# Livioni/OmniVGGT-official

Measured on AMD Instinct MI355X. Metric: frames/sec (518^2, S views) aggregator hot path, higher is better.
Workload: dtype bf16

## Files before the change

### omnivggt-official_amd/build.py

```python
import hashlib
import os
import subprocess
import sys
from concurrent.futures import ThreadPoolExecutor

HERE = os.path.dirname(os.path.abspath(__file__))
CSRC = os.path.join(HERE, "csrc")
OUT = os.path.join(HERE, "libomnivggt_hip.so")
SOURCES = ["ovg_gemm.hip", "ovg_attn.hip", "ovg_elem.hip", "ovg_block.hip", "ovg_head.hip", "ovg_camhead.hip", "ovg_camtab.hip"]
FLAGS = ["--offload-arch=gfx950", "-O3", "-std=c++17", "-fPIC", "-fno-gpu-rdc", "-Wall", "-Wno-unused-function"]
EXTRA_FLAGS = {"ovg_attn.hip": ["-fno-honor-nans"]}


PINNED_ATTENTION_KERNELS = {"IDF16bLi4ELi8ELi0ELi2ELb0ELi5ELi0E": 4, "IDF16bLi4ELi4ELi0ELi2ELb0ELi3ELi0E": 4, "IDF16bLi2ELi4ELi0ELi2ELb0ELi3ELi0E": 2}


PINNED_LOOP_MNEMONICS = {"v_mfma_f32_16x16x32_bf16", "v_exp_f32", "v_cvt_pk_bf16_f32", "ds_read_b128",
                         "v_add_u32_e32", "v_or_b32_e32", "v_lshl_or_b32", "v_lshl_add_u32", "v_add_lshl_u32", "v_lshlrev_b32_e32", "v_and_b32_e32"}


def check_pinned_attention_loops(asm_text):
    import re
    kernels, name, body = {}, None, []
    for line in asm_text.splitlines():
        m = re.match(r"^(_ZN\S*attn16_kernel\S*):", line)
        if m:
            name, body = m.group(1), []
            continue
        if name is not None:
            body.append(line)
            if "s_endpgm" in line:
                kernels[name], name = body, None
    report = {}
    for pat, qb in PINNED_ATTENTION_KERNELS.items():
        hits = [k for k in kernels if pat in k]
        if len(hits) != 1:
            raise RuntimeError("pinned-attention check: kernel %s not found exactly once (%r)" % (pat, hits))
        blocks, cur = [], []
        for line in kernels[hits[0]]:
            if re.match(r"^\.LBB", line):
                blocks.append(cur)
                cur = []
            elif line.startswith("\t") and not line.strip().startswith((".", ";")):
                cur.append(line.split()[0])
        blocks.append(cur)
        pinned = [b for b in blocks if sum("v_mfma" in i for i in b) == 18 * qb and b.count("v_exp_f32") == 16 * qb]
        if len(pinned) != 1:
            raise RuntimeError("pinned-attention check: %s has %d candidate hot loops (MFMA / exp counts per block: %r)"
                               % (pat, len(pinned), [(sum("v_mfma" in i for i in b), b.count("v_exp_f32")) for b in blocks if any("v_mfma" in i for i in b)]))
        hot = pinned[0]
        if hot.count("v_cvt_pk_bf16_f32") != 8 * qb or hot.count("ds_read_b128") != 16:
            raise RuntimeError("pinned-attention check: %s hot loop holds %d converts / %d fragment reads" % (pat, hot.count("v_cvt_pk_bf16_f32"), hot.count("ds_read_b128")))
        bad = [i for i in hot if not (i.startswith("s_") or i in PINNED_LOOP_MNEMONICS)]
        if bad:
            raise RuntimeError("pinned-attention check: hipcc put instructions outside the pinned tile's own set (register copies / spills / "
                               "re-materialised operands) inside the hot loop of %s: %r -- the bf16 attention results of such a build are NOT "
                               "trustworthy" % (pat, sorted(set(bad))))
        report[pat] = {"instructions": len(hot), "mfma": 18 * qb}
    return report

TRANS_OPS = ("v_exp_f32", "v_log_f32", "v_rcp_f32", "v_rsq_f32", "v_sqrt_f32", "v_sin_f32", "v_cos_f32", "v_exp_f16", "v_log_f16", "v_rcp_f16", "v_rsq_f16", "v_sqrt_f16")


def _vregs(operand):
    import re
    out = set()
    for m in re.finditer(r"\bv\[(\d+):(\d+)\]", operand):
        out.update(range(int(m.group(1)), int(m.group(2)) + 1))
    for m in re.finditer(r"\bv(\d+)\b", operand):
        out.add(int(m.group(1)))
    return out


def check_trans_use_in_asm(asm_text):
    seen, in_asm, prev = 0, False, None
    for line in asm_text.splitlines():
        t = line.strip()
        if t.startswith(";;#ASMSTART"):
            in_asm = True
            continue
        if t.startswith(";;#ASMEND"):
            in_asm = False
            continue
        if not line.startswith("\t") or not t or t.startswith((".", ";")):
            if t.endswith(":"):
                prev = None
            continue
        mnem, _, rest = t.partition(" ")
        ops = [o.strip() for o in rest.split(",")]
        if in_asm and prev is not None and (mnem.startswith("v_") or mnem.startswith("ds_") or mnem.startswith("global_") or mnem.startswith("buffer_")):
            seen += 1
            srcs = set()
            for o in (ops[1:] if mnem.startswith("v_") and not mnem.startswith("v_cmp") else ops):
                srcs |= _vregs(o)
            if mnem.startswith("v_fma_mix") or mnem.startswith("v_pk_add") or mnem.startswith("v_mfma"):
                srcs |= _vregs(ops[0])
            if srcs & prev[1]:
                raise RuntimeError("trans-use check: compiler-scheduled %s writes v%s and the inline-asm `%s` directly behind it reads it -- "
                                   "hipcc pads no hazard for asm statements; put an opaque wait state between them (ovg_attn16.h pv_step)"
                                   % (prev[0], sorted(prev[1]), t))
        if mnem == "s_nop":
            prev = None
            continue
        if not in_asm and mnem.split("_e32")[0].split("_e64")[0] in TRANS_OPS:
            prev = (mnem, _vregs(ops[0]))
        else:
            prev = None
    return seen


def _hipcc():
    for c in (os.environ.get("HIPCC"), "/opt/rocm/bin/hipcc", "hipcc"):
        if c and (os.path.isabs(c) and os.path.exists(c) or not os.path.isabs(c)):
            return c
    raise RuntimeError("hipcc not found")


def _digest():
    h = hashlib.sha256()
    files = [os.path.join(CSRC, f) for f in sorted(os.listdir(CSRC))]
    files.append(os.path.join(HERE, "..", "include", "omnivggt_hip.h"))
    for f in files:
        with open(f, "rb") as fh:
            h.update(fh.read())
    h.update(" ".join(FLAGS).encode())
    h.update(repr(sorted(EXTRA_FLAGS.items())).encode())
    return h.hexdigest()


def is_current():
    stamp = OUT + ".stamp"
    return os.path.exists(OUT) and os.path.exists(stamp) and open(stamp).read().strip() == _digest()


def have_hipcc():
    try:
        c = _hipcc()
    except RuntimeError:
        return False
    import shutil
    return os.path.isabs(c) or shutil.which(c) is not None


def build(force=False, verbose=True):
    import fcntl
    import shutil
    import tempfile
    stamp = OUT + ".stamp"
    with open(OUT + ".lock", "w") as lock:
        fcntl.flock(lock, fcntl.LOCK_EX)
        try:
            dig = _digest()
            if not force and is_current():
                return OUT
            hipcc = _hipcc()
            os.makedirs(os.path.join(HERE, "build"), exist_ok=True)
            objdir = tempfile.mkdtemp(prefix="obj.", dir=os.path.join(HERE, "build"))

            def cc(src, extra=()):
                obj = os.path.join(objdir, src.replace(".hip", ".o"))
                cmd = [hipcc, *FLAGS, *EXTRA_FLAGS.get(src, []), *extra, "-c", os.path.join(CSRC, src), "-o", obj]
                if src == "ovg_attn.hip":
                    cmd.insert(1, "-save-temps=obj")
                r = subprocess.run(cmd, capture_output=True, text=True)
                if r.returncode != 0:
                    raise RuntimeError("hipcc failed for %s:\n%s" % (src, r.stderr[-4000:]))
                if verbose and r.stderr.strip():
                    sys.stderr.write(r.stderr)
                if src == "ovg_attn.hip" and not extra:
                    asm = [f for f in os.listdir(objdir) if f.startswith("ovg_attn") and f.endswith(".s") and "gfx950" in f]
                    if len(asm) != 1:
                        raise RuntimeError("pinned-attention check: expected one gfx950 assembly file of ovg_attn.hip, found %r" % asm)
                    try:
                        text = open(os.path.join(objdir, asm[0])).read()
                        check_pinned_attention_loops(text)
                        check_trans_use_in_asm(text)
                    except RuntimeError as e:
                        sys.stderr.write("WARNING: %s\nWARNING: rebuilding ovg_attn.hip with -DOVG_ATTN_PIPE_LOOP=0 (compiler-scheduled attention "
                                         "tile body: correct, slower); fix csrc/ovg_attn16_body_q*.inc for this compiler to get the pinned loop back\n" % e)
                        return cc(src, extra=("-DOVG_ATTN_PIPE_LOOP=0",))
                return obj

            try:
                with ThreadPoolExecutor(max_workers=len(SOURCES)) as ex:
                    objs = list(ex.map(cc, SOURCES))
                tmp_out = os.path.join(objdir, "libomnivggt_hip.so")
                r = subprocess.run([hipcc, "--offload-arch=gfx950", "-shared", "-fPIC", "-o", tmp_out, *objs], capture_output=True, text=True)
                if r.returncode != 0:
                    raise RuntimeError("link failed:\n" + r.stderr[-4000:])
                if os.path.exists(stamp):
                    os.remove(stamp)
                os.replace(tmp_out, OUT)
                with open(stamp + ".tmp", "w") as fh:
                    fh.write(dig)
                os.replace(stamp + ".tmp", stamp)
            finally:
                shutil.rmtree(objdir, ignore_errors=True)
            return OUT
        finally:
            fcntl.flock(lock, fcntl.LOCK_UN)


if __name__ == "__main__":
    print(build(force="--force" in sys.argv))
```

### omnivggt-official_amd/csrc/ovg_gemm.hip

```cpp
#include "ovg_common.h"
#include <mutex>
#include <type_traits>
#include <utility>
#include <vector>

namespace {

constexpr int BM = 128, BN = 128;

#ifdef OVG_GEMM_TIMELINE
__device__ unsigned long long* g_tl_buf = nullptr;
__device__ int g_tl_stagger = 0;
OVG_DEV void tl_mark(int slot) {
  if ((threadIdx.x & 63) != 0 || g_tl_buf == nullptr) return;
  const int wave = threadIdx.x >> 6, last = (blockDim.x >> 6) - 1;
  if (wave != 0 && wave != last) return;
  unsigned long long* row = g_tl_buf + (size_t)blockIdx.x * 16 + (wave == 0 ? 0 : 8);
  row[slot] = wall_clock64();
  if (slot == 0) { row[4] = __builtin_amdgcn_s_getreg((31 << 11) | 4); row[5] = __builtin_amdgcn_s_getreg((31 << 11) | 20); row[6] = clock64(); }
  if (slot == 3) row[7] = clock64();
}
OVG_DEV void tl_stagger() {
  if (g_tl_stagger <= 0 || blockIdx.x >= 256) return;
  const unsigned long long until = wall_clock64() + (unsigned long long)(((blockIdx.x >> 3) & 7) * g_tl_stagger);
// ... 350 lines not shown
        if (m < M) *reinterpret_cast<u32x4*>(static_cast<T*>(p.y) + (int64_t)m * p.ldy + n_w0 + pch * 8) = t[j];
      }
    }
  }
}

template <typename T, int EPI, bool OUT_F32, int MT, int XP = 0, bool X3 = false>
OVG_DEV void linear_epilogue(const ovg_linear_params& p, const f32x4 (&acc)[4][MT], const int m_w0, const int n_w0, const int row_lim = -1) {
  if constexpr (EPI == OVG_EPI_RES) {
    if (p.inject != nullptr) { linear_epilogue_impl<T, EPI, OUT_F32, MT, true, XP, X3>(p, acc, m_w0, n_w0, row_lim); return; }
  }
  linear_epilogue_impl<T, EPI, OUT_F32, MT, false, XP, X3>(p, acc, m_w0, n_w0, row_lim);
}

template <typename T, int EPI, bool OUT_F32, int MT, int XP, bool X3 = false>
OVG_DEV void linear_epilogue_auto(const ovg_linear_params& p, const f32x4 (&acc)[4][MT], const int m_w0, const int n_w0, unsigned char* img) {
  if constexpr (!XP && sizeof(T) == 2) {
    if constexpr ((EPI == OVG_EPI_STORE || EPI == OVG_EPI_GELU) && !OUT_F32 && !X3) {
      if (((p.ldy * (int64_t)sizeof(T)) & 15) == 0) { linear_epilogue_staged<T, EPI, MT>(p, acc, m_w0, n_w0, img); return; }
    }
    if constexpr (EPI == OVG_EPI_RES) {
      bool inj_here = false;
      if (p.inject != nullptr) {
        const int rem = m_w0 % (int)p.inj_period;
        inj_here = rem == 0 || (int)p.inj_period - rem < 16 * MT;
      }
      if (!inj_here) { linear_epilogue_staged<T, EPI, MT>(p, acc, m_w0, n_w0, img); return; }
    }
  }
  linear_epilogue<T, EPI, OUT_F32, MT, XP, X3>(p, acc, m_w0, n_w0);
}


template <typename T, int EPI, bool OUT_F32, int XP = 0, bool X3 = false>
__global__ __launch_bounds__(256, 2) void linear_kernel(ovg_linear_params p, int ntiles_n) {
  __shared__ __attribute__((aligned(16))) unsigned char lds[2 * 128 * 128];
  const int M = (int)p.M, N = (int)p.N, K = (int)p.K;
  int tm, tn;
  tl_stagger();
  tl_mark(0);
  tile_coords(xcd_remap(blockIdx.x, gridDim.x), (M + BM - 1) / BM, ntiles_n, tm, tn);
  const int m0 = tm * BM, n0 = tn * BN;
  f32x4 acc[4][4];
  gemm_mainloop<T, false, X3>(static_cast<const T*>(p.x), p.ldx, static_cast<const T*>(p.w), p.ldw, M, N, K, m0, n0, lds, acc,
                              static_cast<const T*>(p.x_lo), static_cast<const T*>(p.w_lo));
  tl_mark(2);
  const int wave = __builtin_amdgcn_readfirstlane(threadIdx.x >> 6);
  linear_epilogue_auto<T, EPI, OUT_F32, 4, XP, X3>(p, acc, m0 + (wave & 1) * 64, n0 + (wave >> 1) * 64, lds + wave * 8192);
  tl_mark(3);
}

template <typename T, int MT, bool NORM, bool ROPE, bool X3 = false>
OVG_DEV void qk_rows(const f32x4 (&acc)[4][MT], const float* __restrict__ nw_p, const float* __restrict__ nb_p,
                     const float* __restrict__ rope_cos, const float* __restrict__ rope_sin, T* __restrict__ out, const int64_t npad,
                     const int m_w0, const int M, const int seq, const int h, const int tokens_per_view, const int n_special,
                     const int grid_w, const float qk_eps, const float scale, unsigned char* img = nullptr, T* __restrict__ out_lo = nullptr) {
  const int lane = threadIdx.x & 63, g = lane >> 4, lr = lane & 15;
  const FastDiv div_seq(seq), div_tpv(ROPE ? tokens_per_view : 1), div_gw(ROPE ? grid_w : 1);
  float nw[16], nb[16];
  if constexpr (NORM) {
#pragma unroll
    for (int nt = 0; nt < 4; ++nt) {
      const f32x4 a = *reinterpret_cast<const f32x4*>(nw_p + nt * 16 + 4 * g);
      const f32x4 b = *reinterpret_cast<const f32x4*>(nb_p + nt * 16 + 4 * g);
#pragma unroll
      for (int r = 0; r < 4; ++r) { nw[nt * 4 + r] = a[r]; nb[nt * 4 + r] = b[r]; }
    }
  }
#pragma unroll
  for (int mt = 0; mt < MT; ++mt) {
    const int m = m_w0 + mt * 16 + lr;
    const bool valid = m < M;
    const int mm = valid ? m : M - 1;
    int bidx, n;
    div_seq.divmod(mm, bidx, n);
    f32x4 cy, sy, cx, sxn;
    if constexpr (ROPE) {
      int vw, t, py, px;
      div_tpv.divmod(mm, vw, t);
      const int pp = t - n_special;
      div_gw.divmod(pp >= 0 ? pp : 0, py, px);
      py = pp >= 0 ? py + 1 : 0;
      px = pp >= 0 ? px + 1 : 0;
      cy = *reinterpret_cast<const f32x4*>(rope_cos + py * 16 + 4 * g);
      sy = *reinterpret_cast<const f32x4*>(rope_sin + py * 16 + 4 * g);
      cx = *reinterpret_cast<const f32x4*>(rope_cos + px * 16 + 4 * g);
      sxn = *reinterpret_cast<const f32x4*>(rope_sin + px * 16 + 4 * g);
    }
    float v[16];
#pragma unroll
    for (int nt = 0; nt < 4; ++nt)
#pragma unroll
      for (int r = 0; r < 4; ++r) v[nt * 4 + r] = acc[nt][mt][r];
    if constexpr (NORM) {
      float s = 0.f;
#pragma unroll
      for (int i = 0; i < 16; ++i) s += v[i];
      s = quad16_sum(s);
      const float mean = s * (1.0f / 64.0f);
      float q = 0.f;
#pragma unroll
      for (int i = 0; i < 16; ++i) { const float d = v[i] - mean; q += d * d; }
      q = quad16_sum(q);
      float rstd;
      if constexpr (sizeof(T) == 4 || X3) rstd = 1.0f / sqrtf(q * (1.0f / 64.0f) + qk_eps);
      else rstd = __builtin_amdgcn_rsqf(q * (1.0f / 64.0f) + qk_eps);
#pragma unroll
      for (int i = 0; i < 16; ++i) v[i] = (v[i] - mean) * rstd * nw[i] + nb[i];
    }
    if constexpr (ROPE) {
#pragma unroll
      for (int r = 0; r < 4; ++r) {
        const float a0 = v[r], a1 = v[4 + r];
        v[r] = a0 * cy[r] - a1 * sy[r];
        v[4 + r] = a1 * cy[r] + a0 * sy[r];
        const float b0 = v[8 + r], b1 = v[12 + r];
        v[8 + r] = b0 * cx[r] - b1 * sxn[r];
        v[12 + r] = b1 * cx[r] + b0 * sxn[r];
      }
    }
#pragma unroll
    for (int i = 0; i < 16; ++i) v[i] *= scale;
    if constexpr (sizeof(T) == 2) {
      if (img != nullptr) {
#pragma unroll
        for (int nt = 0; nt < 4; ++nt) stage16_put4<T>(img, mt * 16 + lr, nt * 16 + 4 * g, v[nt * 4], v[nt * 4 + 1], v[nt * 4 + 2], v[nt * 4 + 3]);
        continue;
      }
    }
    if (valid) {
      const int64_t off = (((int64_t)bidx * OVG_H + h) * npad + n) * OVG_D + 4 * g;
      T* dst = out + off;
#pragma unroll
      for (int nt = 0; nt < 4; ++nt) {
        if constexpr (X3) store4_hilo(dst + nt * 16, out_lo + off + nt * 16, v[nt * 4], v[nt * 4 + 1], v[nt * 4 + 2], v[nt * 4 + 3]);
        else store4<T>(dst + nt * 16, v[nt * 4], v[nt * 4 + 1], v[nt * 4 + 2], v[nt * 4 + 3]);
      }
    }
  }
  if constexpr (sizeof(T) == 2) {
    if (img != nullptr) {
      const int prow = lane >> 3, pch = lane & 7;
#pragma unroll
      for (int i0 = 0; i0 < 2 * MT; i0 += 4) {
        u32x4 t[4];
#pragma unroll
        for (int j = 0; j < 4; ++j) t[j] = stage16_get(img, (i0 + j) * 8 + prow, pch);
#pragma unroll
        for (int j = 0; j < 4; ++j) {
          const int m = m_w0 + (i0 + j) * 8 + prow;
          int bidx, n;
          div_seq.divmod(m < M ? m : M - 1, bidx, n);
          if (m < M) *reinterpret_cast<u32x4*>(out + (((int64_t)bidx * OVG_H + h) * npad + n) * OVG_D + pch * 8) = t[j];
        }
      }
    }
  }
}

template <typename T, int MT, bool X3 = false>
OVG_DEV void qk_epilogue(const ovg_qkv_params& p, f32x4 (&acc)[4][MT], const int m_w0, const int ncol0_,
                         const float* rope_c, const float* rope_s, unsigned char* img = nullptr) {
  const int ncol0 = __builtin_amdgcn_readfirstlane(ncol0_);
  const int M = (int)p.M;
  const int lane = threadIdx.x & 63, g = lane >> 4;
  const int seq = (int)p.seq;
  const int which = ncol0 / OVG_C;
  const int h = (ncol0 % OVG_C) / OVG_D;

#pragma unroll
  for (int nt = 0; nt < 4; ++nt) {
    const f32x4 b = *reinterpret_cast<const f32x4*>(p.bias + ncol0 + nt * 16 + 4 * g);
#pragma unroll
    for (int mt = 0; mt < MT; ++mt) acc[nt][mt] += b;
  }
  {
    const float* nw_p = which == 0 ? p.qn_w : p.kn_w;
    const float* nb_p = which == 0 ? p.qn_b : p.kn_b;
    T* out = static_cast<T*>(which == 0 ? p.q : p.k);
    T* out_lo = static_cast<T*>(which == 0 ? p.q_lo : p.k_lo);
    const int64_t npad = which == 0 ? p.nq_pad : p.nk_pad;
    const float scale = which == 0 ? p.q_scale : 1.0f;
    const int tpv = (int)p.tokens_per_view;
#define OVG_QK_ROWS(NORM, ROPE) qk_rows<T, MT, NORM, ROPE, X3>(acc, nw_p, nb_p, rope_c, rope_s, out, npad, m_w0, M, seq, h, \
                                                                 tpv, p.n_special, p.grid_w, p.qk_eps, scale, img, out_lo)
    if (p.qk_norm) { if (p.rope) OVG_QK_ROWS(true, true); else OVG_QK_ROWS(true, false); }
    else { if (p.rope) OVG_QK_ROWS(false, true); else OVG_QK_ROWS(false, false); }
#undef OVG_QK_ROWS
  }
}

template <typename T, int MT, bool X3 = false>
OVG_DEV void v_epilogue(const ovg_qkv_params& p, const f32x4 (&acc)[4][MT], const int m_w0, const int ncol0_, const int row_lim = -1) {
  const int ncol0 = __builtin_amdgcn_readfirstlane(ncol0_);
  const int M = row_lim >= 0 ? row_lim : (int)p.M, seq = (int)p.seq;
  const int lane = threadIdx.x & 63, g = lane >> 4, lr = lane & 15;
  const int h = (ncol0 % OVG_C) / OVG_D;
  const FastDiv div_seq(seq);
  float bias[4];
#pragma unroll
  for (int nt = 0; nt < 4; ++nt) bias[nt] = p.bias[ncol0 + nt * 16 + lr];
  T* vt = static_cast<T*>(p.vt);
  const int64_t dlo = X3 ? static_cast<T*>(p.vt_lo) - vt : 0;
#pragma unroll
  for (int mt = 0; mt < MT; ++mt) {
    const int m = m_w0 + mt * 16 + 4 * g;
    const int mc = m < M ? m : M - 1;
    int bidx, n;
    div_seq.divmod(mc, bidx, n);
    const bool inside = (m + 3 < M) && (n + 3 < seq);
    const bool whole = inside && ((n & 3) == 0);
    const bool halves = sizeof(T) == 2 && inside && ((n & 3) == 2);
    T* rowb = vt + (((int64_t)bidx * OVG_H + h) * OVG_D + lr) * p.nk_pad;
    const int c0 = sizeof(T) == 2 ? vt_pos16(n) : n, c2 = sizeof(T) == 2 ? vt_pos16(n + 2) : n + 2;
#pragma unroll
    for (int nt = 0; nt < 4; ++nt) {
      const f32x4 v = acc[nt][mt] + bias[nt];
      T* dst = rowb + (int64_t)nt * 16 * p.nk_pad;
      if (whole) {
        if constexpr (X3) store4_hilo(dst + c0, dst + dlo + c0, v[0], v[1], v[2], v[3]);
        else store4<T>(dst + c0, v[0], v[1], v[2], v[3]);
      } else if (halves) {
        if constexpr (X3) {
          f16_t ph[4], pl[4];
#pragma unroll
          for (int r = 0; r < 4; ++r) split_hilo(v[r], ph[r], pl[r]);
          uint32_t w0, w1, l0, l1;
          __builtin_memcpy(&w0, ph, 4); __builtin_memcpy(&w1, ph + 2, 4);
          __builtin_memcpy(&l0, pl, 4); __builtin_memcpy(&l1, pl + 2, 4);
          *reinterpret_cast<uint32_t*>(dst + c0) = w0;
          *reinterpret_cast<uint32_t*>(dst + c2) = w1;
          *reinterpret_cast<uint32_t*>(dst + dlo + c0) = l0;
          *reinterpret_cast<uint32_t*>(dst + dlo + c2) = l1;
        } else if constexpr (sizeof(T) == 2) {
          T pr[4] = {TT<T>::from_f32(v[0]), TT<T>::from_f32(v[1]), TT<T>::from_f32(v[2]), TT<T>::from_f32(v[3])};
          uint32_t w0, w1;
          __builtin_memcpy(&w0, pr, 4);
          __builtin_memcpy(&w1, pr + 2, 4);
          *reinterpret_cast<uint32_t*>(dst + c0) = w0;
          *reinterpret_cast<uint32_t*>(dst + c2) = w1;
        }
      } else {
#pragma unroll
        for (int r = 0; r < 4; ++r) {
          const int mr = m + r;
          if (mr < M) {
            int br, nr;
            div_seq.divmod(mr, br, nr);
            const int64_t at = (((int64_t)br * OVG_H + h) * OVG_D + nt * 16 + lr) * p.nk_pad + (sizeof(T) == 2 ? vt_pos16(nr) : nr);
            if constexpr (X3) { f16_t eh, el; split_hilo(v[r], eh, el); vt[at] = eh; vt[at + dlo] = el; }
            else vt[at] = TT<T>::from_f32(v[r]);
          }
        }
      }
    }
  }
}

OVG_DEV void stage_rope_table(const ovg_qkv_params& p, unsigned char* tab, int nwaves) {
  if (!p.rope) return;
  typedef __attribute__((address_space(1))) const void* gp_t;
  typedef __attribute__((address_space(3))) void* lp_t;
  const int lane = threadIdx.x & 63;
  const int wave = __builtin_amdgcn_readfirstlane(threadIdx.x >> 6);
  const int bytes = p.max_pos * 64;
  for (int i = wave; i < 16; i += nwaves) {
    const int piece = i & 7;
    int off = piece * 1024 + lane * 16;
    off = off < bytes ? off : bytes - 16;
    const unsigned char* src = reinterpret_cast<const unsigned char*>(i < 8 ? p.rope_cos : p.rope_sin) + off;
    __builtin_amdgcn_global_load_lds((gp_t)src, (lp_t)(tab + i * 1024), 16, 0, 0);
  }
}
constexpr int ROPE_LDS_BYTES = 2 * 128 * 16 * 4;

template <typename T, bool X3 = false>
__global__ __launch_bounds__(256, 3) void qkv_kernel(ovg_qkv_params p, int nt_begin, int nt_count) {
  __shared__ __attribute__((aligned(16))) unsigned char lds[2 * 128 * 128];
  constexpr int N = 3 * OVG_C, K = OVG_C;
  const int M = (int)p.M;
  int tm, tn;
  tl_stagger();
  tl_mark(0);
  tile_coords(xcd_remap(blockIdx.x, gridDim.x), (M + BM - 1) / BM, nt_count, tm, tn);
  const int m0 = tm * BM, n0 = (nt_begin + tn) * BN;
  const int wave = threadIdx.x >> 6;
  f32x4 acc[4][4];
  if (n0 >= 2 * OVG_C) {
    gemm_mainloop<T, true, X3>(static_cast<const T*>(p.x), p.ldx, static_cast<const T*>(p.w), (int64_t)K, M, N, K, m0, n0, lds, acc,
                               static_cast<const T*>(p.x_lo), static_cast<const T*>(p.w_lo));
    tl_mark(2);
    v_epilogue<T, 4, X3>(p, acc, m0 + (wave & 1) * 64, n0 + (wave >> 1) * 64);
  } else {
    gemm_mainloop<T, false, X3>(static_cast<const T*>(p.x), p.ldx, static_cast<const T*>(p.w), (int64_t)K, M, N, K, m0, n0, lds, acc,
                                static_cast<const T*>(p.x_lo), static_cast<const T*>(p.w_lo));
    tl_mark(2);
    unsigned char* img = (sizeof(T) == 2 && !X3 && !(p.tile & OVG_TILE_R02_EPILOGUE)) ? lds + __builtin_amdgcn_readfirstlane(wave) * 8192 : nullptr;
    qk_epilogue<T, 4, X3>(p, acc, m0 + (wave & 1) * 64, n0 + (wave >> 1) * 64, p.rope_cos, p.rope_sin, img);
  }
  tl_mark(3);
}

#include "ovg_gemm256.h"

template <typename T, int EPI, bool OUT_F32, int XP = 0, bool X3 = false>
__global__ __launch_bounds__(512) void linear256_kernel(ovg_linear_params p, int ntiles_n) {
  extern __shared__ __attribute__((aligned(16))) unsigned char lds256[];
  const int M = (int)p.M, N = (int)p.N, K = (int)p.K;
  int tm, tn;
  tl_stagger();
  tl_mark(0);
  tile_coords(xcd_remap(blockIdx.x, gridDim.x), (M + g256::BM2 - 1) / g256::BM2, ntiles_n, tm, tn);
  const int m0 = tm * g256::BM2, n0 = tn * g256::BN2;
  f32x4 acc[4][8];
  g256::mainloop<T, false, X3>(static_cast<const T*>(p.x), p.ldx, static_cast<const T*>(p.w), p.ldw, M, N, K, m0, n0, lds256, acc,
                                static_cast<const T*>(p.x_lo), static_cast<const T*>(p.w_lo));
  tl_mark(2);
  const int wave = __builtin_amdgcn_readfirstlane(threadIdx.x >> 6);
  linear_epilogue_auto<T, EPI, OUT_F32, 8, XP, X3>(p, acc, m0 + (wave >> 2) * 128, n0 + (wave & 3) * 64, lds256 + wave * 16384);
  tl_mark(3);
}

template <typename T, bool X3 = false>
__global__ __launch_bounds__(512) void qkv256_kernel(ovg_qkv_params p, int nt_begin, int nt_count) {
  extern __shared__ __attribute__((aligned(16))) unsigned char lds256[];
  constexpr int N = 3 * OVG_C, K = OVG_C;
  const int M = (int)p.M;
  int tm, tn;
  tl_stagger();
  tl_mark(0);
  tile_coords(xcd_remap(blockIdx.x, gridDim.x), (M + g256::BM2 - 1) / g256::BM2, nt_count, tm, tn);
  const int m0 = tm * g256::BM2, n0 = (nt_begin + tn) * g256::BN2;
  const int wave = threadIdx.x >> 6;
  f32x4 acc[4][8];
  if (n0 >= 2 * OVG_C) {
    g256::mainloop<T, true, X3>(static_cast<const T*>(p.x), p.ldx, static_cast<const T*>(p.w), (int64_t)K, M, N, K, m0, n0, lds256, acc,
                                 static_cast<const T*>(p.x_lo), static_cast<const T*>(p.w_lo));
    tl_mark(2);
    v_epilogue<T, 8, X3>(p, acc, m0 + (wave >> 2) * 128, n0 + (wave & 3) * 64);
  } else {
    float* rope_tab = reinterpret_cast<float*>(lds256 + g256::LDS_BYTES);
    stage_rope_table(p, lds256 + g256::LDS_BYTES, 8);
    g256::mainloop<T, false, X3>(static_cast<const T*>(p.x), p.ldx, static_cast<const T*>(p.w), (int64_t)K, M, N, K, m0, n0, lds256, acc,
                                  static_cast<const T*>(p.x_lo), static_cast<const T*>(p.w_lo));
    unsigned char* img = (X3 || (p.tile & OVG_TILE_R02_EPILOGUE)) ? nullptr : lds256 + __builtin_amdgcn_readfirstlane(wave) * 16384;
    tl_mark(2);
    qk_epilogue<T, 8, X3>(p, acc, m0 + (wave >> 2) * 128, n0 + (wave & 3) * 64, rope_tab, rope_tab + 128 * 16, img);
  }
  tl_mark(3);
}

template <typename KernelT>
int allow_big_lds(KernelT kernel, int bytes = g256::LDS_BYTES) {
  static std::mutex mu;
  static std::vector<std::pair<const void*, int>> done;
  const void* fn = reinterpret_cast<const void*>(kernel);
  int dev = 0;
  if (hipGetDevice(&dev) != hipSuccess) return OVG_E_LAUNCH;
  std::lock_guard<std::mutex> lock(mu);
  for (const auto& d : done)
    if (d.first == fn && d.second == dev) return OVG_OK;
  if (hipFuncSetAttribute(fn, hipFuncAttributeMaxDynamicSharedMemorySize, bytes) != hipSuccess) return OVG_E_LAUNCH;
  done.emplace_back(fn, dev);
  return OVG_OK;
}

constexpr int TILE_GROUP = 8, TILE_GROUP256 = 4;

bool aligned16(const void* p) { return (reinterpret_cast<uintptr_t>(p) & 15) == 0; }

template <typename T, int XP>
int launch_linear128_xp(const ovg_linear_params& p, hipStream_t st) {
  const int mt = (int)((p.M + BM - 1) / BM), nt = (int)(p.N / BN);
  const dim3 grid(mt * nt), block(256);
  const int ntg = nt | (TILE_GROUP << 16);
  switch (p.epilogue) {
    case OVG_EPI_STORE:
      if (p.out_f32) OVG_LAUNCH((linear_kernel<T, OVG_EPI_STORE, true, XP>), grid, block, 0, st, p, ntg);
      else OVG_LAUNCH((linear_kernel<T, OVG_EPI_STORE, false, XP>), grid, block, 0, st, p, ntg);
      break;
    case OVG_EPI_GELU:
      OVG_LAUNCH((linear_kernel<T, OVG_EPI_GELU, false, XP>), grid, block, 0, st, p, ntg);
      break;
    case OVG_EPI_RES:
      OVG_LAUNCH((linear_kernel<T, OVG_EPI_RES, true, XP>), grid, block, 0, st, p, ntg);
      break;
    case OVG_EPI_PATCH:
      OVG_LAUNCH((linear_kernel<T, OVG_EPI_PATCH, true, XP>), grid, block, 0, st, p, ntg);
      break;
    default: return OVG_E_ARG;
  }
  OVG_CHECK_LAUNCH();
  return OVG_OK;
}
template <typename T>
int launch_linear128(const ovg_linear_params& p, hipStream_t st) {
  if constexpr (sizeof(T) == 2) {
#ifdef OVG_AB_VARIANTS
    if (p.tile & OVG_TILE_R02_EPILOGUE) return launch_linear128_xp<T, 1>(p, st);
#else
    if (p.tile & OVG_TILE_R02_EPILOGUE) return OVG_E_UNSUPPORTED;
#endif
  }
  return launch_linear128_xp<T, 0>(p, st);
}
template <typename T, int EPI, bool OUT_F32, int XP = 0>
int launch_linear256_one(const ovg_linear_params& p, hipStream_t st) {
  const int ok = allow_big_lds(linear256_kernel<T, EPI, OUT_F32, XP>);
  if (ok != OVG_OK) return ok;
  const int mt = (int)((p.M + g256::BM2 - 1) / g256::BM2), nt = (int)(p.N / g256::BN2);
  const int ntg = nt | (TILE_GROUP256 << 16);
  OVG_LAUNCH((linear256_kernel<T, EPI, OUT_F32, XP>), dim3(mt * nt), dim3(512), g256::LDS_BYTES, st, p, ntg);
  OVG_CHECK_LAUNCH();
  return OVG_OK;
}
template <typename T>
int launch_linear256(const ovg_linear_params& p, hipStream_t st, bool xp) {
#ifdef OVG_AB_VARIANTS
  if (xp) {
    switch (p.epilogue) {
      case OVG_EPI_STORE: return p.out_f32 ? launch_linear256_one<T, OVG_EPI_STORE, true>(p, st) : launch_linear256_one<T, OVG_EPI_STORE, false, 1>(p, st);
      case OVG_EPI_GELU: return launch_linear256_one<T, OVG_EPI_GELU, false, 1>(p, st);
      case OVG_EPI_RES: return launch_linear256_one<T, OVG_EPI_RES, true, 1>(p, st);
      case OVG_EPI_PATCH: return launch_linear256_one<T, OVG_EPI_PATCH, true>(p, st);
      default: return OVG_E_ARG;
    }
  }
#else
  if (xp) return OVG_E_UNSUPPORTED;
#endif
  switch (p.epilogue) {
    case OVG_EPI_STORE: return p.out_f32 ? launch_linear256_one<T, OVG_EPI_STORE, true>(p, st) : launch_linear256_one<T, OVG_EPI_STORE, false>(p, st);
    case OVG_EPI_GELU: return launch_linear256_one<T, OVG_EPI_GELU, false>(p, st);
    case OVG_EPI_RES: return launch_linear256_one<T, OVG_EPI_RES, true>(p, st);
    case OVG_EPI_PATCH: return launch_linear256_one<T, OVG_EPI_PATCH, true>(p, st);
    default: return OVG_E_ARG;
  }
}
#ifndef OVG_PROJ_256_ONE_ROUND
#define OVG_PROJ_256_ONE_ROUND 1
#endif
int gemm_device_cus() {
  static const int n = [] {
    int dev = 0, v = 0;
    if (hipGetDevice(&dev) != hipSuccess || hipDeviceGetAttribute(&v, hipDeviceAttributeMultiprocessorCount, dev) != hipSuccess || v <= 0) v = 256;
    return v;
  }();
  return n;
}
int choose_256(int tile_arg, bool sixteen_bit, int64_t M, int64_t N, int64_t K, bool light_epilogue_or_long_k, int kind = 0) {
  const int tile = tile_arg & ~OVG_TILE_R02_EPILOGUE;
  const bool legal = sixteen_bit && N % g256::BN2 == 0 && K % 64 == 0;
  if (tile == OVG_TILE_128) return 0;
  if (tile == OVG_TILE_256) return legal ? 1 : -1;
  if (tile != OVG_TILE_AUTO) return -1;
  if (!legal) return 0;
  if (M >= 20000) return light_epilogue_or_long_k ? 1 : 0;
  const int64_t cus = gemm_device_cus();
  const int64_t t256 = ((M + 255) / 256) * (N / 256), t128 = ((M + 127) / 128) * (N / 128);
  if (kind == 2 && M >= 8000 && t256 <= cus) return 1;
  if (OVG_PROJ_256_ONE_ROUND && kind == 3 && t256 <= cus && t128 > 3 * cus) return 1;
  return 0;
}

template <typename T>
int launch_linear(const ovg_linear_params& p, hipStream_t st) {
  const int big = choose_256(p.tile, sizeof(T) == 2, p.M, p.N, p.K, p.epilogue != OVG_EPI_RES || p.K >= 2048,
                             p.epilogue == OVG_EPI_GELU ? 1 : (p.epilogue == OVG_EPI_RES ? (p.K >= 2048 ? 2 : 3) : 0));
  if (big < 0) return OVG_E_ARG;
  if constexpr (sizeof(T) == 2) {
    if (big) return launch_linear256<T>(p, st, (p.tile & OVG_TILE_R02_EPILOGUE) != 0);
  }
  return launch_linear128<T>(p, st);
}

template <int EPI, bool OUT_F32>
int launch_linear_x3_one(const ovg_linear_params& p, hipStream_t st, bool big) {
  if (big) {
    const int ok = allow_big_lds(linear256_kernel<f16_t, EPI, OUT_F32, 0, true>);
    if (ok != OVG_OK) return ok;
    const int mt = (int)((p.M + g256::BM2 - 1) / g256::BM2), nt = (int)(p.N / g256::BN2);
    OVG_LAUNCH((linear256_kernel<f16_t, EPI, OUT_F32, 0, true>), dim3(mt * nt), dim3(512), g256::LDS_BYTES, st, p, nt | (TILE_GROUP256 << 16));
  } else {
    const int mt = (int)((p.M + BM - 1) / BM), nt = (int)(p.N / BN);
    OVG_LAUNCH((linear_kernel<f16_t, EPI, OUT_F32, 0, true>), dim3(mt * nt), dim3(256), 0, st, p, nt | (TILE_GROUP << 16));
  }
  OVG_CHECK_LAUNCH();
  return OVG_OK;
}
int launch_linear_x3(const ovg_linear_params& p, hipStream_t st) {
  int big = choose_256(p.tile, true, p.M, p.N, p.K, true);
  if (big < 0) return OVG_E_ARG;
  switch (p.epilogue) {
    case OVG_EPI_STORE: return p.out_f32 ? launch_linear_x3_one<OVG_EPI_STORE, true>(p, st, big) : launch_linear_x3_one<OVG_EPI_STORE, false>(p, st, big);
    case OVG_EPI_GELU: return launch_linear_x3_one<OVG_EPI_GELU, false>(p, st, big);
    case OVG_EPI_RES: return launch_linear_x3_one<OVG_EPI_RES, true>(p, st, big);
    case OVG_EPI_PATCH: return launch_linear_x3_one<OVG_EPI_PATCH, true>(p, st, big);
    default: return OVG_E_ARG;
  }
}

#ifdef OVG_GEMM_TIMELINE
}
extern "C" int ovg_lab_gemm_timeline(void* buf, int stagger_ticks) {
  unsigned long long* b = static_cast<unsigned long long*>(buf);
  if (hipMemcpyToSymbol(HIP_SYMBOL(g_tl_buf), &b, sizeof(b)) != hipSuccess) return OVG_E_LAUNCH;
  if (hipMemcpyToSymbol(HIP_SYMBOL(g_tl_stagger), &stagger_ticks, sizeof(int)) != hipSuccess) return OVG_E_LAUNCH;
  return OVG_OK;
}
namespace {
#endif

}

extern "C" int ovg_linear(const ovg_linear_params* p, void* stream) {
  if (!p || !p->x || !p->w || !p->y) return OVG_E_ARG;
  if (p->M <= 0 || p->N <= 0 || p->K <= 0 || p->M > (1 << 30)) return OVG_E_ARG;
  if (p->N % BN != 0 || p->K % 64 != 0) return OVG_E_ARG;
  const int64_t esz = p->dtype == OVG_F32 ? 4 : 2;
  if ((p->ldx * esz) % 16 || (p->ldw * esz) % 16 || !aligned16(p->x) || !aligned16(p->w) || !aligned16(p->y)) return OVG_E_ARG;
  if (p->bias && !aligned16(p->bias)) return OVG_E_ARG;
  if (p->epilogue == OVG_EPI_RES) {
    if (!p->res || !p->gamma || (p->ldres % 4) || (p->ldy % 4) || !aligned16(p->res) || !aligned16(p->gamma)) return OVG_E_ARG;
    if (p->inject && (p->inj_period <= 0 || !aligned16(p->inject))) return OVG_E_ARG;
  } else if (p->epilogue == OVG_EPI_PATCH) {
    if (!p->table || p->p0 <= 0 || p->p1 <= 0 || (p->ldy % 4) || !aligned16(p->table)) return OVG_E_ARG;
  } else {
    const int64_t osz = p->out_f32 ? 4 : esz;
    if ((p->ldy * osz) % (4 * osz)) return OVG_E_ARG;
  }
  hipStream_t st = static_cast<hipStream_t>(stream);
  switch (p->dtype) {
    case OVG_BF16: return launch_linear<bf16_t>(*p, st);
    case OVG_F16: return launch_linear<f16_t>(*p, st);
    case OVG_F32: return launch_linear<float>(*p, st);
    case OVG_F16X2: {
      if (!p->x_lo || !p->w_lo || !aligned16(p->x_lo) || !aligned16(p->w_lo)) return OVG_E_ARG;
      const bool out16 = (p->epilogue == OVG_EPI_STORE || p->epilogue == OVG_EPI_GELU) && !p->out_f32;
      if (out16 && (!p->y_lo || !aligned16(p->y_lo))) return OVG_E_ARG;
      return launch_linear_x3(*p, st);
    }
    default: return OVG_E_DTYPE;
  }
}

extern "C" int ovg_qkv(const ovg_qkv_params* p, void* stream) {
  if (!p || !p->x || !p->w || !p->bias || !p->q || !p->k || !p->vt) return OVG_E_ARG;
  if (p->M <= 0 || p->M > (1 << 30) || p->seq <= 0 || p->M % p->seq != 0) return OVG_E_ARG;
  if (p->nq_pad < p->seq || p->nk_pad < p->seq || p->nk_pad % OVG_KV_TILE != 0) return OVG_E_ARG;
  if (p->dtype != OVG_BF16 && p->dtype != OVG_F16 && p->dtype != OVG_F32 && p->dtype != OVG_F16X2) return OVG_E_DTYPE;
  const int64_t esz = p->dtype == OVG_F32 ? 4 : 2;
  if ((p->ldx * esz) % 16 || !aligned16(p->x) || !aligned16(p->w) || !aligned16(p->bias) || !aligned16(p->q) || !aligned16(p->k) || !aligned16(p->vt)) return OVG_E_ARG;
  if (p->dtype == OVG_F16X2) {
    if (!p->x_lo || !p->w_lo || !aligned16(p->x_lo) || !aligned16(p->w_lo)) return OVG_E_ARG;
    if ((p->part != 2 && (!p->k_lo || !p->vt_lo || !aligned16(p->k_lo) || !aligned16(p->vt_lo))) || (p->part != 1 && (!p->q_lo || !aligned16(p->q_lo)))) return OVG_E_ARG;
  }
  if (p->qk_norm && (!p->qn_w || !p->qn_b || !p->kn_w || !p->kn_b)) return OVG_E_ARG;
  if (p->rope) {
    if (!p->rope_cos || !p->rope_sin || p->tokens_per_view <= 0 || p->grid_w <= 0) return OVG_E_ARG;
    const int64_t np = p->tokens_per_view - p->n_special;
    if (np <= 0 || (np - 1) / p->grid_w + 1 >= p->max_pos || p->grid_w >= p->max_pos) return OVG_E_ARG;
    if (p->max_pos > 128 || !aligned16(p->rope_cos) || !aligned16(p->rope_sin)) return OVG_E_ARG;
  }
  if (p->part < 0 || p->part > 2) return OVG_E_ARG;
  hipStream_t st = static_cast<hipStream_t>(stream);
  const int big = choose_256(p->tile, p->dtype != OVG_F32, p->M, (p->part == 0 ? 3 : (p->part == 1 ? 2 : 1)) * OVG_C, OVG_C, true);
  if (big < 0) return OVG_E_ARG;
  if (big) {
    const int q_t = OVG_C / g256::BN2, all_t = 3 * OVG_C / g256::BN2;
    const int ntb = p->part == 1 ? q_t : 0;
    const int ntc = p->part == 0 ? all_t : (p->part == 1 ? all_t - q_t : q_t);
    const dim3 grid2((unsigned)(((p->M + g256::BM2 - 1) / g256::BM2) * ntc));
    const int ntg2 = ntc | (TILE_GROUP256 << 16);
    if (p->dtype == OVG_BF16) {
      const int ok = allow_big_lds(qkv256_kernel<bf16_t>, g256::LDS_BYTES + ROPE_LDS_BYTES);
      if (ok != OVG_OK) return ok;
      OVG_LAUNCH((qkv256_kernel<bf16_t>), grid2, dim3(512), g256::LDS_BYTES + ROPE_LDS_BYTES, st, *p, ntb, ntg2);
    } else if (p->dtype == OVG_F16X2) {
      const int ok = allow_big_lds(qkv256_kernel<f16_t, true>, g256::LDS_BYTES + ROPE_LDS_BYTES);
      if (ok != OVG_OK) return ok;
      OVG_LAUNCH((qkv256_kernel<f16_t, true>), grid2, dim3(512), g256::LDS_BYTES + ROPE_LDS_BYTES, st, *p, ntb, ntg2);
    } else {
      const int ok = allow_big_lds(qkv256_kernel<f16_t>, g256::LDS_BYTES + ROPE_LDS_BYTES);
      if (ok != OVG_OK) return ok;
      OVG_LAUNCH((qkv256_kernel<f16_t>), grid2, dim3(512), g256::LDS_BYTES + ROPE_LDS_BYTES, st, *p, ntb, ntg2);
    }
    OVG_CHECK_LAUNCH();
    return OVG_OK;
  }
  const int q_tiles = OVG_C / BN, all_tiles = 3 * OVG_C / BN;
  const int nt_begin = p->part == 1 ? q_tiles : 0;
  const int nt_count = p->part == 0 ? all_tiles : (p->part == 1 ? all_tiles - q_tiles : q_tiles);
  const dim3 grid((unsigned)(((p->M + BM - 1) / BM) * nt_count)), block(256);
  const int ntg = nt_count | (TILE_GROUP << 16);
  switch (p->dtype) {
    case OVG_BF16: OVG_LAUNCH((qkv_kernel<bf16_t>), grid, block, 0, st, *p, nt_begin, ntg); break;
    case OVG_F16: OVG_LAUNCH((qkv_kernel<f16_t>), grid, block, 0, st, *p, nt_begin, ntg); break;
    case OVG_F16X2: OVG_LAUNCH((qkv_kernel<f16_t, true>), grid, block, 0, st, *p, nt_begin, ntg); break;
    default: OVG_LAUNCH((qkv_kernel<float>), grid, block, 0, st, *p, nt_begin, ntg); break;
  }
  OVG_CHECK_LAUNCH();
  return OVG_OK;
}
```

Before: 80.79.

## Add 4-wave 256x256 GEMM variant with AGPR accumulators for large residual projections

Adds a 256-thread linear256 kernel in which each wave owns a 128x128 output sub-tile held in AGPR accumulators. It uses hand-scheduled MFMA, LDS fragment reads and DMA staging in a double-buffered register loop, and runs the epilogue in two halves. Large-M residual-epilogue GEMMs (the attention and MLP output projections) are routed to the 256 tile path and this 4-wave kernel. The aim is more operand reuse per wave and less LDS traffic per MFMA. The cost is one wave per SIMD occupancy and a build-time assembly check that rejects spills or stray instructions in the hot loop.

```diff
diff --git a/omnivggt-official_amd/build.py b/omnivggt-official_amd/build.py
--- a/omnivggt-official_amd/build.py
+++ b/omnivggt-official_amd/build.py
@@ -59,6 +59,55 @@
         report[pat] = {"instructions": len(hot), "mfma": 18 * qb}
     return report
 
+GEMM_W4_KERNEL = r"^(_Z\S*linear256_kernelI\S*Lb0ELb1EEEv\S*):"
+GEMM_W4_LOOP_MNEMONICS = {"v_mfma_f32_16x16x32_bf16", "v_mfma_f32_16x16x32_f16", "ds_read_b128", "global_load_lds_dwordx4",
+                          "v_add_u32_e32", "v_add3_u32", "v_or_b32_e32", "v_lshl_or_b32", "v_lshl_add_u32", "v_add_lshl_u32", "v_lshlrev_b32_e32",
+                          "v_and_b32_e32", "v_xor_b32_e32"}
+
+
+def check_gemm_w4_loops(asm_text):
+    import re
+    kernels, name, body = {}, None, []
+    for line in asm_text.splitlines():
+        m = re.match(GEMM_W4_KERNEL, line)
+        if m:
+            name, body = m.group(1), []
+            continue
+        if name is not None:
+            body.append(line)
+            if "s_endpgm" in line:
+                kernels[name], name = body, None
+    if not kernels:
+        raise RuntimeError("gemm-w4 check: no 4-wave linear256 kernel found")
+    report = {}
+    for k, lines in kernels.items():
+        blocks, cur = [], []
+        for line in lines:
+            if re.match(r"^(\.LBB|; %bb\.)", line):
+                blocks.append(cur)
+                cur = []
+            elif line.startswith("\t") and not line.strip().startswith((".", ";")):
+                cur.append(line.split()[0])
+        blocks.append(cur)
+        if any(i.startswith("scratch_") for b in blocks for i in b):
+            raise RuntimeError("gemm-w4 check: %s accesses scratch (spilled accumulators or registers)" % k)
+        hot = [b for b in blocks if any(i.startswith("v_mfma") for i in b) and "global_load_lds_dwordx4" in b]
+        if len(hot) != 1:
+            raise RuntimeError("gemm-w4 check: %s has %d steady-state loops, expected 1" % (k, len(hot)))
+        b = hot[0]
+        st = b.count("s_barrier")
+        mf = sum(i.startswith("v_mfma") for i in b)
+        if st < 1 or mf != 64 * st or b.count("ds_read_b128") != 16 * st or b.count("global_load_lds_dwordx4") != 8 * st:
+            raise RuntimeError("gemm-w4 check: %s loop holds %d MFMAs / %d fragment reads / %d DMA requests over %d k-stages (want 64 / 16 / 8 each)"
+                               % (k, mf, b.count("ds_read_b128"), b.count("global_load_lds_dwordx4"), st))
+        bad = [i for i in b if not (i.startswith("s_") or i in GEMM_W4_LOOP_MNEMONICS)]
+        if bad:
+            raise RuntimeError("gemm-w4 check: hipcc put instructions outside the loop's own set (accumulator copies / spills / moves) into the "
+                               "hot loop of %s: %r" % (k, sorted(set(bad))))
+        report[k] = {"k_stages": st, "mfma": mf, "instructions": len(b)}
+    return report
+
+
 TRANS_OPS = ("v_exp_f32", "v_log_f32", "v_rcp_f32", "v_rsq_f32", "v_sqrt_f32", "v_sin_f32", "v_cos_f32", "v_exp_f16", "v_log_f16", "v_rcp_f16", "v_rsq_f16", "v_sqrt_f16")
 
 
@@ -160,13 +209,18 @@
             def cc(src, extra=()):
                 obj = os.path.join(objdir, src.replace(".hip", ".o"))
                 cmd = [hipcc, *FLAGS, *EXTRA_FLAGS.get(src, []), *extra, "-c", os.path.join(CSRC, src), "-o", obj]
-                if src == "ovg_attn.hip":
+                if src in ("ovg_attn.hip", "ovg_gemm.hip"):
                     cmd.insert(1, "-save-temps=obj")
                 r = subprocess.run(cmd, capture_output=True, text=True)
                 if r.returncode != 0:
                     raise RuntimeError("hipcc failed for %s:\n%s" % (src, r.stderr[-4000:]))
                 if verbose and r.stderr.strip():
                     sys.stderr.write(r.stderr)
+                if src == "ovg_gemm.hip":
+                    asm = [f for f in os.listdir(objdir) if f.startswith("ovg_gemm") and f.endswith(".s") and "gfx950" in f]
+                    if len(asm) != 1:
+                        raise RuntimeError("gemm-w4 check: expected one gfx950 assembly file of ovg_gemm.hip, found %r" % asm)
+                    check_gemm_w4_loops(open(os.path.join(objdir, asm[0])).read())
                 if src == "ovg_attn.hip" and not extra:
                     asm = [f for f in os.listdir(objdir) if f.startswith("ovg_attn") and f.endswith(".s") and "gfx950" in f]
                     if len(asm) != 1:
diff --git a/omnivggt-official_amd/csrc/ovg_gemm.hip b/omnivggt-official_amd/csrc/ovg_gemm.hip
--- a/omnivggt-official_amd/csrc/ovg_gemm.hip
+++ b/omnivggt-official_amd/csrc/ovg_gemm.hip
@@ -676,9 +676,19 @@
 }
 
 #include "ovg_gemm256.h"
-
-template <typename T, int EPI, bool OUT_F32, int XP = 0, bool X3 = false>
-__global__ __launch_bounds__(512) void linear256_kernel(ovg_linear_params p, int ntiles_n) {
+#include "ovg_gemm256w4.h"
+
+#if defined(OVG_AB_VARIANTS) && defined(OVG_GEMM256_W8)
+constexpr bool kGemm256W4 = false;
+#else
+constexpr bool kGemm256W4 = true;
+#endif
+constexpr int threads256(bool w4) { return w4 ? g256w4::THREADS : 512; }
+constexpr int waves256(bool w4) { return w4 ? 1 : 2; }
+
+template <typename T, int EPI, bool OUT_F32, int XP = 0, bool X3 = false, bool W4 = false>
+__global__ __launch_bounds__(threads256(W4)) __attribute__((amdgpu_waves_per_eu(waves256(W4), waves256(W4))))
+void linear256_kernel(ovg_linear_params p, int ntiles_n) {
   extern __shared__ __attribute__((aligned(16))) unsigned char lds256[];
   const int M = (int)p.M, N = (int)p.N, K = (int)p.K;
   int tm, tn;
@@ -686,12 +696,23 @@
   tl_mark(0);
   tile_coords(xcd_remap(blockIdx.x, gridDim.x), (M + g256::BM2 - 1) / g256::BM2, ntiles_n, tm, tn);
   const int m0 = tm * g256::BM2, n0 = tn * g256::BN2;
-  f32x4 acc[4][8];
-  g256::mainloop<T, false, X3>(static_cast<const T*>(p.x), p.ldx, static_cast<const T*>(p.w), p.ldw, M, N, K, m0, n0, lds256, acc,
-                                static_cast<const T*>(p.x_lo), static_cast<const T*>(p.w_lo));
-  tl_mark(2);
   const int wave = __builtin_amdgcn_readfirstlane(threadIdx.x >> 6);
-  linear_epilogue_auto<T, EPI, OUT_F32, 8, XP, X3>(p, acc, m0 + (wave >> 2) * 128, n0 + (wave & 3) * 64, lds256 + wave * 16384);
+  if constexpr (W4) {
+    static_assert(!X3 && !XP, "the split-f16 kernels and the r02 epilogue forms stay on the 8-wave loop");
+    f32x4 acc[8][8];
+    g256w4::mainloop<T>(static_cast<const T*>(p.x), p.ldx, static_cast<const T*>(p.w), p.ldw, M, N, K, m0, n0, lds256, acc);
+    tl_mark(2);
+    const int m_w0 = m0 + (wave >> 1) * 128, n_w0 = n0 + (wave & 1) * 128;
+    unsigned char* img = lds256 + wave * 32768;
+    linear_epilogue_auto<T, EPI, OUT_F32, 8, XP, X3>(p, g256w4::half_cols<0>(acc), g256w4::opaque(m_w0), n_w0, img);
+    linear_epilogue_auto<T, EPI, OUT_F32, 8, XP, X3>(p, g256w4::half_cols<1>(acc), g256w4::opaque(m_w0), n_w0 + 64, img + 16384);
+  } else {
+    f32x4 acc[4][8];
+    g256::mainloop<T, false, X3>(static_cast<const T*>(p.x), p.ldx, static_cast<const T*>(p.w), p.ldw, M, N, K, m0, n0, lds256, acc,
+                                  static_cast<const T*>(p.x_lo), static_cast<const T*>(p.w_lo));
+    tl_mark(2);
+    linear_epilogue_auto<T, EPI, OUT_F32, 8, XP, X3>(p, acc, m0 + (wave >> 2) * 128, n0 + (wave & 3) * 64, lds256 + wave * 16384);
+  }
   tl_mark(3);
 }
 
@@ -778,16 +799,17 @@
   }
   return launch_linear128_xp<T, 0>(p, st);
 }
-template <typename T, int EPI, bool OUT_F32, int XP = 0>
+template <typename T, int EPI, bool OUT_F32, int XP = 0, bool W4 = false>
 int launch_linear256_one(const ovg_linear_params& p, hipStream_t st) {
-  const int ok = allow_big_lds(linear256_kernel<T, EPI, OUT_F32, XP>);
+  const int ok = allow_big_lds(linear256_kernel<T, EPI, OUT_F32, XP, false, W4>);
   if (ok != OVG_OK) return ok;
   const int mt = (int)((p.M + g256::BM2 - 1) / g256::BM2), nt = (int)(p.N / g256::BN2);
   const int ntg = nt | (TILE_GROUP256 << 16);
-  OVG_LAUNCH((linear256_kernel<T, EPI, OUT_F32, XP>), dim3(mt * nt), dim3(512), g256::LDS_BYTES, st, p, ntg);
+  OVG_LAUNCH((linear256_kernel<T, EPI, OUT_F32, XP, false, W4>), dim3(mt * nt), dim3(threads256(W4)), g256::LDS_BYTES, st, p, ntg);
   OVG_CHECK_LAUNCH();
   return OVG_OK;
 }
+bool choose_w4(const ovg_linear_params& p) { return kGemm256W4 && p.epilogue == OVG_EPI_RES && p.M >= 20000; }
 template <typename T>
 int launch_linear256(const ovg_linear_params& p, hipStream_t st, bool xp) {
 #ifdef OVG_AB_VARIANTS
@@ -806,11 +828,15 @@
   switch (p.epilogue) {
     case OVG_EPI_STORE: return p.out_f32 ? launch_linear256_one<T, OVG_EPI_STORE, true>(p, st) : launch_linear256_one<T, OVG_EPI_STORE, false>(p, st);
     case OVG_EPI_GELU: return launch_linear256_one<T, OVG_EPI_GELU, false>(p, st);
-    case OVG_EPI_RES: return launch_linear256_one<T, OVG_EPI_RES, true>(p, st);
+    case OVG_EPI_RES:
+      return choose_w4(p) ? launch_linear256_one<T, OVG_EPI_RES, true, 0, true>(p, st) : launch_linear256_one<T, OVG_EPI_RES, true>(p, st);
     case OVG_EPI_PATCH: return launch_linear256_one<T, OVG_EPI_PATCH, true>(p, st);
     default: return OVG_E_ARG;
   }
 }
+#ifndef OVG_PROJ_256_W4
+#define OVG_PROJ_256_W4 1
+#endif
 #ifndef OVG_PROJ_256_ONE_ROUND
 #define OVG_PROJ_256_ONE_ROUND 1
 #endif
@@ -829,7 +855,7 @@
   if (tile == OVG_TILE_256) return legal ? 1 : -1;
   if (tile != OVG_TILE_AUTO) return -1;
   if (!legal) return 0;
-  if (M >= 20000) return light_epilogue_or_long_k ? 1 : 0;
+  if (M >= 20000) return (light_epilogue_or_long_k || (OVG_PROJ_256_W4 && kind == 3)) ? 1 : 0;
   const int64_t cus = gemm_device_cus();
   const int64_t t256 = ((M + 255) / 256) * (N / 256), t128 = ((M + 127) / 128) * (N / 128);
   if (kind == 2 && M >= 8000 && t256 <= cus) return 1;
diff --git a/omnivggt-official_amd/csrc/ovg_gemm256w4.h b/omnivggt-official_amd/csrc/ovg_gemm256w4.h
--- /dev/null
+++ b/omnivggt-official_amd/csrc/ovg_gemm256w4.h
@@ -0,0 +1,118 @@
+#pragma once
+
+namespace g256w4 {
+
+using g256::ROWB;
+using g256::SLOTS;
+using g256::STAGE_B;
+using g256::W_TILE;
+using g256::swz64;
+constexpr int NP = 8;
+constexpr int THREADS = 256;
+
+template <typename T> OVG_DEV void mma_agpr(f32x4& c, const u32x4& a, const u32x4& b) {
+  if constexpr (std::is_same<T, bf16_t>::value) asm volatile("v_mfma_f32_16x16x32_bf16 %0, %1, %2, %0" : "+a"(c) : "v"(a), "v"(b));
+  else asm volatile("v_mfma_f32_16x16x32_f16 %0, %1, %2, %0" : "+a"(c) : "v"(a), "v"(b));
+}
+OVG_DEV void settle_acc() { asm volatile("s_nop 7\n\ts_nop 7\n\ts_nop 3" ::: "memory"); }
+
+OVG_DEV void wait_stages_in_flight(int n) {
+  if (n >= 3) asm volatile("s_waitcnt vmcnt(24)" ::: "memory");
+  else if (n == 2) asm volatile("s_waitcnt vmcnt(16)" ::: "memory");
+  else if (n == 1) asm volatile("s_waitcnt vmcnt(8)" ::: "memory");
+  else asm volatile("s_waitcnt vmcnt(0)" ::: "memory");
+}
+
+template <typename T>
+OVG_DEV void mainloop(const T* __restrict__ X, int64_t ldx, const T* __restrict__ W, int64_t ldw,
+                      int M, int N, int K, int m0, int n0, unsigned char* lds, f32x4 (&acc)[8][8]) {
+  static_assert(sizeof(T) == 2, "16-bit operands");
+  const int tid = threadIdx.x, lane = tid & 63;
+  const int wave = __builtin_amdgcn_readfirstlane(tid >> 6);
+  const int wn = wave & 1, wm = wave >> 1;
+  const int g = lane >> 4, lr = lane & 15;
+
+  const unsigned char* wbase = reinterpret_cast<const unsigned char*>(W + (int64_t)n0 * ldw);
+  const unsigned char* xbase = reinterpret_cast<const unsigned char*>(X + (int64_t)m0 * ldx);
+  uint32_t wg[4], xg[4];
+#pragma unroll
+  for (int i = 0; i < 4; ++i) {
+    const int row = wave * 64 + i * 16 + (lane >> 2);
+    const int wr = n0 + row < N ? row : N - 1 - n0;
+    const int xr = m0 + row < M ? row : M - 1 - m0;
+    const uint32_t ch = (uint32_t)(((lane & 3) ^ swz64(row)) * 16);
+    wg[i] = (uint32_t)wr * (uint32_t)(ldw * 2) + ch;
+    xg[i] = (uint32_t)xr * (uint32_t)(ldx * 2) + ch;
+  }
+  const int nk = (K * 2) / ROWB;
+  const uint32_t lds_base = __builtin_amdgcn_readfirstlane((uint32_t)(uintptr_t)lds);
+  auto stage_piece = [&](int kt, int j) {
+    const uint32_t sb = lds_base + (kt & (SLOTS - 1)) * STAGE_B + wave * 64 * ROWB;
+    const int64_t ko = (int64_t)kt * ROWB;
+    if (j < 4) lds_dma16_s(wbase + ko, wg[j], sb + j * 16 * ROWB);
+    else lds_dma16_s(xbase + ko, xg[j - 4], sb + W_TILE + (j - 4) * 16 * ROWB);
+  };
+#pragma unroll
+  for (int a = 0; a < 8; ++a)
+#pragma unroll
+    for (int b = 0; b < 8; ++b) acc[a][b] = f32x4{0.f, 0.f, 0.f, 0.f};
+
+  const int frag_off = lr * ROWB + (g ^ swz64(lr)) * 16;
+  const unsigned char* wfrag = lds + wn * 128 * ROWB + frag_off;
+  const unsigned char* xfrag = lds + W_TILE + wm * 128 * ROWB + frag_off;
+  u32x4 a0[8], a1[8], b[8];
+
+  for (int s = 0; s < SLOTS; ++s)
+    if (s < nk)
+      for (int j = 0; j < NP; ++j) stage_piece(s, j);
+  wait_stages_in_flight((nk < SLOTS ? nk : SLOTS) - 1);
+  __builtin_amdgcn_s_barrier();
+  tl_mark(1);
+#pragma unroll
+  for (int t = 0; t < 8; ++t) a0[t] = *reinterpret_cast<const u32x4*>(wfrag + t * 16 * ROWB);
+#pragma unroll
+  for (int t = 0; t < 8; ++t) b[t] = *reinterpret_cast<const u32x4*>(xfrag + t * 16 * ROWB);
+  __builtin_amdgcn_sched_barrier(0);
+
+  auto body = [&](int t, const u32x4 (&acur)[8], u32x4 (&anxt)[8], bool dma, int infl) __attribute__((always_inline)) {
+    asm volatile("s_waitcnt lgkmcnt(0)" ::: "memory");
+    if (infl >= 0) wait_stages_in_flight(infl);
+    __builtin_amdgcn_s_barrier();
+    __builtin_amdgcn_sched_barrier(0);
+    const int so = ((t + 1) & (SLOTS - 1)) * STAGE_B;
+    const unsigned char* wn_ = wfrag + so;
+    const unsigned char* xn_ = xfrag + so;
+#pragma unroll
+    for (int mt = 0; mt < 8; ++mt) {
+#pragma unroll
+      for (int nt = 0; nt < 8; ++nt) mma_agpr<T>(acc[nt][mt], acur[nt], b[mt]);
+      anxt[mt] = *reinterpret_cast<const u32x4*>(wn_ + mt * 16 * ROWB);
+      b[mt] = *reinterpret_cast<const u32x4*>(xn_ + mt * 16 * ROWB);
+      __builtin_amdgcn_sched_barrier(0);
+      if (dma) { stage_piece(t + SLOTS, mt); __builtin_amdgcn_sched_barrier(0); }
+    }
+  };
+
+  int t = 0;
+  for (; t + SLOTS + 1 < nk; t += 2) {
+    body(t, a0, a1, true, SLOTS - 2);
+    body(t + 1, a1, a0, true, SLOTS - 2);
+  }
+  for (; t + 1 < nk; t += 2) {
+    const int i0 = nk - 2 - t, i1 = nk - 3 - t;
+    body(t, a0, a1, false, i0 < SLOTS - 2 ? i0 : SLOTS - 2);
+    body(t + 1, a1, a0, false, i1 < 0 ? -1 : (i1 < SLOTS - 2 ? i1 : SLOTS - 2));
+  }
+  asm volatile("s_waitcnt lgkmcnt(0)" ::: "memory");
+  settle_acc();
+  __builtin_amdgcn_s_barrier();
+}
+
+template <int H> OVG_DEV f32x4 (&half_cols(f32x4 (&acc)[8][8]))[4][8] { return *reinterpret_cast<f32x4(*)[4][8]>(&acc[4 * H]); }
+
+OVG_DEV int opaque(int v) {
+  asm volatile("" : "+s"(v));
+  return v;
+}
+
+}
```

After: 81.02 (median of 6 runs). Within noise of the previous version (+0.3%).
